# sabbirhossainujjal/LLMVoX

Hardware: AMD Instinct MI355X
Metric: speech tokens/sec (+ 24kHz audio samples/sec = 320 x tokens/s; p50 first-chunk latency) (higher is better)
Workload: dtype bf16

## Files before the change

### llmvox_amd/csrc/ar_kernels.hip

```cpp
#include "ar_plan.h"

#pragma clang fp contract(off)

namespace lvx {

#ifdef LVX_TIMING
constexpr int TS_BLOCKS = 1024;
__device__ uint64_t g_lvx_ts[16 * 4 * TS_BLOCKS * 4];
#define TS_DECL uint64_t ts_[2] = {0, 0}
#define TS_MARK(i) do { if (threadIdx.x == 0) ts_[i] = __builtin_amdgcn_s_memrealtime(); } while (0)
#define TS_SAVE(tag, layer, blk)                                                                    \
  do {                                                                                               \
    if (threadIdx.x == 0) {                                                                          \
      const uint64_t te_ = __builtin_amdgcn_s_memrealtime();                                         \
      const uint64_t hw_ = (uint64_t)__builtin_amdgcn_s_getreg((31 << 11) | 4) |                    \
                           ((uint64_t)__builtin_amdgcn_s_getreg((3 << 11) | 20) << 32);              \
      uint64_t* p_ = g_lvx_ts + ((size_t)(((tag) * 4 + (layer)) * TS_BLOCKS + min((int)(blk), TS_BLOCKS - 1))) * 4; \
      p_[0] = ts_[0]; p_[1] = ts_[1]; p_[2] = te_; p_[3] = hw_;                                      \
    }                                                                                                \
  } while (0)
#else
#define TS_DECL do {} while (0)
#define TS_MARK(i) do {} while (0)
#define TS_SAVE(tag, layer, blk) do {} while (0)
// ... 908 lines not shown
__device__ __forceinline__ void slot_update_bf16(float& m, float& l, f32x2_t (&o)[12], float sc, const uint4 (&vp)[3],
                                                 bool valid) {
  uint32_t v[12];
#pragma unroll
  for (int i = 0; i < 3; ++i) { v[4 * i] = vp[i].x; v[4 * i + 1] = vp[i].y; v[4 * i + 2] = vp[i].z; v[4 * i + 3] = vp[i].w; }
  if (!valid) return;
  const float mn = fmaxf(m, sc);
  const float alpha = __builtin_amdgcn_exp2f((m - mn) * 1.4426950408889634f);
  const float p = __builtin_amdgcn_exp2f((sc - mn) * 1.4426950408889634f);
  l = l * alpha + p;
  const f32x2_t a2 = f32x2_t{alpha, alpha}, p2 = f32x2_t{p, p};
#pragma unroll
  for (int j = 0; j < 12; ++j) {
    const f32x2_t vv = f32x2_t{__uint_as_float(v[j] << 16), __uint_as_float(v[j] & 0xffff0000u)};
    o[j] = __builtin_elementwise_fma(p2, vv, o[j] * a2);
  }
  m = mn;
}
__device__ __forceinline__ void slot_softmax_step_bf16(float& m, float& l, f32x2_t (&o)[12], const QSplit& qs,
                                                       const uint4 (&kp)[3], const uint4 (&vp)[3], bool valid) {
  slot_update_bf16(m, l, o, slot_score_bf16(qs, kp), vp, valid);
}

__device__ __forceinline__ float slot_fold_wave(float m, float& l, float (&o)[24]) {
  const float M = wave_max(m);
  const float f = (m == -INFINITY) ? 0.f : expf(m - M);
  l *= f;
#pragma unroll
  for (int i = 0; i < 24; ++i) o[i] *= f;
  return M;
}

__device__ __forceinline__ float4 q0_row_stats(const GemvArgs& a, int4 rn, int b, int lane, bool store_x);
__device__ __forceinline__ int l0_next_tok(const ArState& st, int jn, int loaded) {
  if (!st.text_plan) return 384;
  return (jn + 1 < st.plan_stride) ? min(max(loaded, 0), TEXT_VOCAB - 1) : -1;
}
__device__ __forceinline__ void lds_barrier() {
  asm volatile("s_waitcnt lgkmcnt(0)" ::: "memory");
  __builtin_amdgcn_s_barrier();
  asm volatile("" ::: "memory");
}

template <typename TKV, int DEPTH, int NW, bool QKV, bool L0>
__device__ __forceinline__ void attn_v2_body(const ArState st, int layer, int ns_max, int direct, int selcopy,
                                             const GemvArgs* a0) {
  constexpr int TK = NW * 16;
  constexpr bool SLOT = sizeof(TKV) < 4;
  static_assert(!QKV || (NW == 4 && sizeof(TKV) == 4), "the K-split c_attn: the fp32 parity mode's 4-wave blocks");
  static_assert(!L0 || (NW == 4 && SLOT && !QKV), "the fused layer-0 form: bf16 / fp8 KV in 4-wave blocks");
  constexpr bool NEWKV = QKV || L0;
  constexpr int QH = NEWKV ? (3 * HD + NW * 64 - 1) / (NW * 64) : 1;
  __shared__ float wm_s[NW], wl_s[NW];
  __shared__ float wo_s[NW][4][HD];
  __shared__ float qs_s[NEWKV ? HD : 1];
  __shared__ __attribute__((aligned(16))) TKV kvh_s[NEWKV ? 2 : 1][NEWKV ? HD : 1];
  __shared__ float sv_s[L0 ? 4 : 1], sv2_s[L0 ? 4 : 1];
  __shared__ int si_s[L0 ? 4 : 1];
  __shared__ float4 sst_s;
  const int sp = blockIdx.x, head = blockIdx.y, b = blockIdx.z;
  const int tid = threadIdx.x, wave = tid >> 6, lane = tid & 63;
  TS_DECL;
  TS_MARK(0);
  int4 rold = make_int4(-1, 0, 0, 0);
  int2 rx = make_int2(0, 0);
  bool tk = false;
  float4 lgv[L0 ? VOCAB / 1024 : 1];
  int zn[L0 ? QH : 1];
  float zg[L0 ? QH : 1], zt[L0 ? QH : 1], zp[L0 ? QH : 1];
  int jnx = 0, tnext = 384;
  int4 ri0 = make_int4(-1, 0, 0, 0);
  if constexpr (L0) {
    rold = st.rowinfo[b];
    rx = st.rowx[b];
    const unsigned pend = st.selrow[b];
    const float4* lg = reinterpret_cast<const float4*>(st.logits + (size_t)b * VOCAB);
#pragma unroll
    for (int k = 0; k < VOCAB / 1024; ++k) lgv[k] = lg[k * 256 + tid];
#pragma unroll
    for (int h = 0; h < QH; ++h) {
      const int e = min(tid + NW * 64 * h, 3 * HD - 1);
      zn[h] = (e / HD) * D + head * HD + e % HD;
      zg[h] = a0->q0_g[zn[h]];
    }
    tk = pend && rold.x >= 0;
    const int p1 = min(max(tk ? rold.y + 1 : rold.y, 0), st.max_pos - 1);
    const int t1 = tk ? rx.y : rold.z;
#pragma unroll
    for (int h = 0; h < QH; ++h) {
      zt[h] = a0->q0_text[(size_t)(t1 < 0 ? 384 : t1) * (3 * D) + zn[h]];
      zp[h] = a0->q0_pos[(size_t)p1 * (3 * D) + zn[h]];
    }
    jnx = tk ? rx.x + 1 : rx.x;
    if (st.text_plan) tnext = st.text_plan[(size_t)b * st.plan_stride + min(jnx + 1, st.plan_stride - 1)];
    ri0 = make_int4(rold.x, p1, 0, 0);
    if (rold.x < 0) {
      if (head == 0) {
        if (tid == 0) {
          st.rowinfo_n[b] = rold;
          st.rowx_n[b] = make_int2(jnx, l0_next_tok(st, jnx, tnext));
        }
        if (tid < D / 4) reinterpret_cast<float4*>(st.x + (size_t)b * D)[tid] = make_float4(0.f, 0.f, 0.f, 0.f);
      }
      return;
    }
  }
  const int4 ri = L0 ? ri0 : selcopy ? st.rowinfo_n[b] : st.rowinfo[b];
  float pq[QH][QKV ? 4 : 1];
  if constexpr (QKV) {
#pragma unroll
    for (int h = 0; h < QH; ++h) {
      const int e = min(tid + NW * 64 * h, 3 * HD - 1);
      const float* pp = st.qkvp + (size_t)b * (3 * D) + (e / HD) * D + head * HD + e % HD;
#pragma unroll
      for (int k = 0; k < 4; ++k) pq[h][k] = pp[(size_t)k * st.max_streams * (3 * D)];
    }
  }
  const bool cp = selcopy && sp == 0 && head == 0 && tid == 0;
  int jn = 0;
  if (cp) {
    jn = st.rowx_n[b].x;
    st.rowinfo[b] = ri;
    st.selrow[b] = 1u;
    if (b == 0) *st.selp = 0u;
  }
  auto copy_tail = [&]() {
    if (cp) st.rowx[b] = make_int2(jn, plan_tok(st, b, jn + 1));
  };
  const int s = ri.x;
  if (s < 0) {
    copy_tail();
    if (direct == ATTN_F32_ROWS && sp == 0 && tid < HD) st.part_o[(size_t)(b * N_HEAD + head) * NSPLIT * HD + tid] = 0.f;
    return;
  }
  const int t = ri.y + 1;
  const int ns = min(ns_max, (t + ATK - 1) / ATK);
  if (sp >= ns) return;
  const int chunk = SLOT ? (((t + ns - 1) / ns + ATK - 1) / ATK) * ATK : (t + ns - 1) / ns;
  const int k0 = sp * chunk, k1 = L0 ? t - 1 : min(t, k0 + chunk);
  const size_t base = kv_at(layer, st.kv_chunks, st.max_streams, s, head, 0);
  const size_t cstride = (size_t)st.max_streams * N_HEAD * KV_CHUNK * HD;
  const TKV* __restrict__ Kg = reinterpret_cast<const TKV*>(st.kc) + base;
  const TKV* __restrict__ Vg = reinterpret_cast<const TKV*>(st.vc) + base;
  auto krow = [&](int k) { return (size_t)(k / KV_CHUNK) * cstride + (size_t)(k % KV_CHUNK) * HD; };
  const int part = tid & 3, kq = tid >> 2;
  float q[24];
  if constexpr (!NEWKV) {
    const float* qg = st.q + (size_t)b * D + head * HD + part * 24;
#pragma unroll
    for (int i = 0; i < 24; i += 4) {
      const float4 v = *reinterpret_cast<const float4*>(qg + i);
      q[i] = v.x * 0.10206207261596575f; q[i + 1] = v.y * 0.10206207261596575f;
      q[i + 2] = v.z * 0.10206207261596575f; q[i + 3] = v.w * 0.10206207261596575f;
    }
  }
  float m = -INFINITY, l = 0.f, o[24];
#pragma unroll
  for (int i = 0; i < 24; ++i) o[i] = 0.f;
  KvPiece<TKV> kpr[DEPTH][3], vpr[DEPTH][3];
  const int klast = ((k1 - 1) / ATK) * ATK;
  auto issue = [&](int kb, KvPiece<TKV>(&kp)[3], KvPiece<TKV>(&vp)[3]) {
    if constexpr (SLOT) {
      const size_t off = (size_t)min((kb / KV_CHUNK) + (kq / KV_CHUNK), klast / KV_CHUNK) * cstride +
                         (size_t)(kq % KV_CHUNK) * HD + part * 24;
#pragma unroll
      for (int i = 0; i < 3; ++i) {
        kp[i].load(Kg + off + i * 8);
        vp[i].load(Vg + off + i * 8);
      }
      return;
    }
    const int key = min(kb + kq, k1 - 1);
// ... 51 lines not shown
    const float alpha = (m == -INFINITY) ? 0.f : expf(m - mn);
    const float p = valid ? expf(sc - mn) : 0.f;
    l = l * alpha + wave_sum(part == 0 ? p : 0.f);
#pragma unroll
    for (int i = 0; i < 24; ++i) o[i] = fmaf(valid ? p : 0.f, valid ? vf[i] : 0.f, o[i] * alpha);
    m = mn;
  };
#pragma unroll
  for (int d = 0; d < DEPTH; ++d) issue(k0 + d * TK, kpr[d], vpr[d]);
  if constexpr (QKV) {
#pragma unroll
    for (int h = 0; h < QH; ++h) {
      const int e = tid + NW * 64 * h;
      float v = 0.f;
#pragma unroll
      for (int k = 0; k < 4; ++k) v += pq[h][k];
      if (e < HD) {
        qs_s[e] = v;
      } else if (e < 3 * HD && k1 == t) {
        const int which = e / HD - 1, d = e % HD;
        TKV hv;
        if constexpr (sizeof(TKV) == 4) hv = v;
        else if constexpr (sizeof(TKV) == 2) hv = f32_to_bf16(v);
        else hv = f32_to_fp8(v);
        kvh_s[which][d] = hv;
        reinterpret_cast<TKV*>(which ? st.vc : st.kc)[base + krow(ri.y) + d] = hv;
      }
    }
    asm volatile("s_waitcnt lgkmcnt(0)" ::: "memory");
    __builtin_amdgcn_s_barrier();
    asm volatile("" ::: "memory");
#pragma unroll
    for (int i = 0; i < 24; ++i) q[i] = qs_s[part * 24 + i] * 0.10206207261596575f;
  }
  if constexpr (L0) {
    const GemvArgs& a = *a0;
    Best bt{-INFINITY, -INFINITY, 0x7fffffff};
#pragma unroll
    for (int k = 0; k < VOCAB / 1024; ++k) {
      const int i0 = (k * 256 + tid) * 4;
      bt = best_merge(bt, Best{lgv[k].x, -INFINITY, i0});
      bt = best_merge(bt, Best{lgv[k].y, -INFINITY, i0 + 1});
      bt = best_merge(bt, Best{lgv[k].z, -INFINITY, i0 + 2});
      bt = best_merge(bt, Best{lgv[k].w, -INFINITY, i0 + 3});
    }
    bt = best_wave(bt);
    if (lane == 0) { sv_s[wave] = bt.v; sv2_s[wave] = bt.v2; si_s[wave] = bt.i; }
    lds_barrier();
    int4 rn = rold;
    if (tk) {
      Best r{sv_s[0], sv2_s[0], si_s[0]};
#pragma unroll
      for (int w = 1; w < 4; ++w) r = best_merge(r, Best{sv_s[w], sv2_s[w], si_s[w]});
      r = softmax_ties(st.logits + (size_t)b * VOCAB, r, lane);
      const int sl = rold.x, p = rold.y + 1, j = rx.x;
      rn = make_int4(sl, min(p, st.max_pos - 1), rx.y, min(max(r.i, 0), VOCAB - 1));
      if (head == 0 && tid == 0) {
        if (p >= st.max_pos) atomicOr(st.err, 1);
        if (j < st.plan_stride) {
          st.tok_plan[(size_t)b * st.plan_stride + j] = r.i;
          if (st.margin_plan) st.margin_plan[(size_t)b * st.plan_stride + j] = r.v - r.v2;
        }
        st.prev[sl] = r.i;
        st.pos[sl] = p;
        st.rowstep[b] = j + 1;
      }
// ... 12 lines not shown
    lds_barrier();
    const float4 ss = sst_s;
    const float cz = rn.y == 0 ? 0.f : 1.f;
#pragma unroll
    for (int h = 0; h < QH; ++h) {
      const int e = tid + NW * 64 * h;
      const float v = ss.z * (((zt[h] + cz * zc[h]) * ss.x + zp[h]) - ss.y * zg[h]);
      if (e < HD) {
        qs_s[e] = v;
      } else if (e < 3 * HD) {
        const int which = e / HD - 1, d = e % HD;
        TKV hv;
        if constexpr (sizeof(TKV) == 2) hv = f32_to_bf16(v);
        else hv = f32_to_fp8(v);
        kvh_s[which][d] = hv;
        reinterpret_cast<TKV*>(which ? st.vc : st.kc)[base + krow(ri.y) + d] = hv;
      }
    }
    lds_barrier();
#pragma unroll
    for (int i = 0; i < 24; ++i) q[i] = qs_s[part * 24 + i] * 0.10206207261596575f;
    TS_MARK(1);
  }
  if constexpr (BF) qsplit_make(q, qsp);
  for (int kb = k0; kb < k1; kb += DEPTH * TK) {
#pragma unroll
    for (int d = 0; d < DEPTH; ++d) {
      if (DEPTH == 2 && d > 0 && kb + d * TK >= k1) break;
      tile(kb + d * TK, kpr[d], vpr[d]);
      issue(kb + (d + DEPTH) * TK, kpr[d], vpr[d]);
      if (DEPTH > 2) __builtin_amdgcn_sched_barrier(0);
    }
  }
  if constexpr (L0) {
    const bool mine = kq == (t - 1) % TK;
    KvPiece<TKV> kx[3], vx[3];
#pragma unroll
    for (int i = 0; i < 3; ++i) {
      kx[i].load(kvh_s[0] + part * 24 + i * 8);
      vx[i].load(kvh_s[1] + part * 24 + i * 8);
    }
    if constexpr (BF) {
      uint4 ku[3], vu[3];
#pragma unroll
      for (int i = 0; i < 3; ++i) { ku[i] = reinterpret_cast<const uint4&>(kx[i]); vu[i] = reinterpret_cast<const uint4&>(vx[i]); }
      slot_softmax_step_bf16(m, l, o2, qsp, ku, vu, mine);
    } else {
      float kf[24], vf[24];
#pragma unroll
      for (int i = 0; i < 3; ++i) { kx[i].get(kf + 8 * i); vx[i].get(vf + 8 * i); }
      slot_softmax_step(m, l, o, q, kf, vf, mine);
    }
    TS_SAVE(9, layer, head + N_HEAD * b);
  }
  if constexpr (BF) {
#pragma unroll
    for (int j = 0; j < 12; ++j) { o[2 * j] = o2[j].x; o[2 * j + 1] = o2[j].y; }
  }
  if constexpr (SLOT) {
    m = slot_fold_wave(m, l, o);
    l = wave_sum(part == 0 ? l : 0.f);
  }
#pragma unroll
  for (int i = 0; i < 24; ++i) {
    float v = o[i];
    v += dpp_f32<0x128>(v);
    v += dpp_f32<0x124>(v);
// ... 15 lines not shown
    float ov = 0.f, lv = 0.f;
#pragma unroll
    for (int w = 0; w < NW; ++w) {
      const float f = (wm_s[w] == -INFINITY) ? 0.f : expf(wm_s[w] - M);
      ov += f * ((wo_s[w][0][tid] + wo_s[w][1][tid]) + (wo_s[w][2][tid] + wo_s[w][3][tid]));
      lv += f * wl_s[w];
    }
    if (direct == ATTN_F32_ROWS) {
      st.part_o[(size_t)(b * N_HEAD + head) * NSPLIT * HD + tid] = ov * (1.0f / lv);
      return;
    }
    if (direct) {
      st.xn[direct == ATTN_XN_PACKED ? xfrag(b, head * HD + tid, D) : (size_t)b * D + head * HD + tid] = f32_to_bf16(ov * (1.0f / lv));
      return;
    }
    st.part_o[((size_t)(b * N_HEAD + head) * NSPLIT + sp) * HD + tid] = ov;
    if (tid == 0) {
      float* ml = st.part_ml + ((size_t)(b * N_HEAD + head) * NSPLIT + sp) * 2;
      ml[0] = M;
      ml[1] = lv;
    }
  }
}

template <typename TKV, int DEPTH, int NW, bool QKV = false>
__global__ __launch_bounds__(NW * 64) void ar_attn_v2_kernel(ArState st, int layer, int ns_max, int direct,
                                                         int selcopy) {
  attn_v2_body<TKV, DEPTH, NW, QKV, false>(st, layer, ns_max, direct, selcopy, nullptr);
}

template <typename TKV>
__global__ __launch_bounds__(256) LVX_LOADS_FIRST void ar_attn_l0_kernel(GemvArgs a, int direct) {
  attn_v2_body<TKV, 2, 4, false, true>(a.st, 0, 1, direct, 0, &a);
}

__device__ __forceinline__ void hist_store(const ArState& st, int s, int p, int tok) {
  if (st.rowstep && p < st.max_pos) st.hist[(size_t)s * st.max_pos + p] = (uint16_t)tok;
}

template <bool HIST = false>
__device__ __forceinline__ void argmax_row(const ArState& st, int b, int4 ri, float* sv, float* sv2, int* si) {
  const int tid = threadIdx.x, wave = tid >> 6, lane = tid & 63;
  const float4* lg = reinterpret_cast<const float4*>(st.logits + (size_t)b * VOCAB);
  Best bt{-INFINITY, -INFINITY, 0x7fffffff};
#pragma unroll
  for (int j = 0; j < VOCAB / 1024; ++j) {
    const float4 v = lg[j * 256 + tid];
    const int i0 = (j * 256 + tid) * 4;
    bt = best_merge(bt, Best{v.x, -INFINITY, i0});
    bt = best_merge(bt, Best{v.y, -INFINITY, i0 + 1});
    bt = best_merge(bt, Best{v.z, -INFINITY, i0 + 2});
    bt = best_merge(bt, Best{v.w, -INFINITY, i0 + 3});
  }
  bt = best_wave(bt);
  if (lane == 0) { sv[wave] = bt.v; sv2[wave] = bt.v2; si[wave] = bt.i; }
  __syncthreads();
  if (wave == 0) {
    Best r{sv[0], sv2[0], si[0]};
    for (int w = 1; w < 4; ++w) r = best_merge(r, Best{sv[w], sv2[w], si[w]});
    r = softmax_ties(st.logits + (size_t)b * VOCAB, r, lane);
    if (lane == 0) {
      argmax_commit(st, b, ri, r);
      if constexpr (HIST) hist_store(st, ri.x, ri.y, r.i);
    }
  }
}
// ... 236 lines not shown
  if (tid == 0) {
    first = min(min(wfirst[0], wfirst[1]), min(wfirst[2], wfirst[3]));
    last = max(max(wlast[0], wlast[1]), max(wlast[2], wlast[3]));
    r.i = first != 0x7fffffff ? first : max(last, 0);
    hist_store(st, s, ri.y, r.i);
    argmax_commit(st, b, ri, r);
  }
}


template <typename TW, int K, int KW, int RPW, int IN, int OUT>
static void launch_gemv(const GemvArgs& a, hipStream_t s) {
  const int rows_per_block = (4 / KW) * RPW;
  dim3 grid((a.N + rows_per_block - 1) / rows_per_block);
  constexpr int BGMAX = (K == 768) ? 16 : 4;
  if constexpr (OUT == GOUT_LOGITS_GRAN || IN == GIN_EMBED_SELECT) {
    if (a.B <= 1) hipLaunchKernelGGL((ar_gemv_kernel<TW, K, KW, RPW, 1, IN, OUT>), grid, dim3(256), 0, s, a);
    else if (a.B <= 2) hipLaunchKernelGGL((ar_gemv_kernel<TW, K, KW, RPW, 2, IN, OUT>), grid, dim3(256), 0, s, a);
    else hipLaunchKernelGGL((ar_gemv_kernel<TW, K, KW, RPW, 4, IN, OUT>), grid, dim3(256), 0, s, a);
  } else {
    if constexpr (IN == GIN_MERGE && OUT == GOUT_RESID && K == 768 && KW == 1) {
      if (a.B == 1) {
        hipLaunchKernelGGL((ar_cproj_b1_kernel<TW, RPW, NSPLIT>), grid, dim3(256), 0, s, a);
        return;
      }
    }
    if (a.B <= 1) hipLaunchKernelGGL((ar_gemv_kernel<TW, K, KW, RPW, 1, IN, OUT>), grid, dim3(256), 0, s, a);
    else if (a.B <= 2) hipLaunchKernelGGL((ar_gemv_kernel<TW, K, KW, RPW, 2, IN, OUT>), grid, dim3(256), 0, s, a);
    else if (a.B <= 4 || BGMAX == 4) hipLaunchKernelGGL((ar_gemv_kernel<TW, K, KW, RPW, 4, IN, OUT>), grid, dim3(256), 0, s, a);
    else if (a.B <= 8) hipLaunchKernelGGL((ar_gemv_kernel<TW, K, KW, RPW, (BGMAX >= 8 ? 8 : 4), IN, OUT>), grid, dim3(256), 0, s, a);
    else hipLaunchKernelGGL((ar_gemv_kernel<TW, K, KW, RPW, BGMAX, IN, OUT>), grid, dim3(256), 0, s, a);
  }
}

typedef __bf16 bf16x8_t __attribute__((ext_vector_type(8)));
typedef float f32x4_t __attribute__((ext_vector_type(4)));

__device__ __forceinline__ uint2 pack4_bf16(float4 v) {
  return make_uint2((uint32_t)f32_to_bf16(v.x) | ((uint32_t)f32_to_bf16(v.y) << 16),
                    (uint32_t)f32_to_bf16(v.z) | ((uint32_t)f32_to_bf16(v.w) << 16));
}

#ifndef LVX_YCS
#define LVX_YCS 2
#endif
constexpr int YCS = LVX_YCS;

__device__ __forceinline__ void embed_row(const GemvArgs& a, int4 ri, int lane, float4 (&v)[3], float* rden = nullptr) {
  if (ri.x < 0) {
#pragma unroll
    for (int j = 0; j < 3; ++j) v[j] = make_float4(0.f, 0.f, 0.f, 0.f);
    return;
  }
  const int p = ri.y, prev = ri.w;
  const int tok = ri.z < 0 ? 384 : ri.z;
  float4 pe[3];
  const float* wr_ = a.wpe + (size_t)p * D;
#pragma unroll
  for (int j = 0; j < 3; ++j) pe[j] = *reinterpret_cast<const float4*>(wr_ + j * 256 + lane * 4);
#pragma unroll
  for (int j = 0; j < 3; ++j) {
    const int k = j * 256 + lane * 4;
    v[j] = j == 0 ? *reinterpret_cast<const float4*>(a.text_table + (size_t)tok * TEXT_DIM + k)
                  : *reinterpret_cast<const float4*>(a.codebook + (size_t)prev * SPEECH_DIM + (k - TEXT_DIM));
  }
  if (ri.z < 0 && lane == 0) atomicOr(a.st.err, 2);
  float ss = 0.f;
#pragma unroll
  for (int j = 0; j < 3; ++j) {
// ... 397 lines not shown
  const int B = a.B;
  TS_DECL;
  TS_MARK(0);
  const bf16_t* __restrict__ X = XM == M2X_LN_AFTER ? a.st.xb : ((KTOT == 768) ? a.st.xn : a.st.hb);
  const int k0 = by * K + wave * 192 + 8 * (lane >> 4);
  constexpr int EPT = (16 * NT * 16 + NW * 64 - 1) / (NW * 64);
  static_assert((NW * 64) % (NT * 16) == 0, "one batch row per thread in the epilogue");
  int4 ripre = make_int4(-1, 0, 0, 0);
  float xpre[(OUT == M2OUT_RESID_STATS || OUT == M2OUT_RESID) ? EPT : 1];
  float gpre[(OUT == M2OUT_RESID_STATS || XM == M2X_LN_AFTER) ? EPT : 1];
  if constexpr (OUT == M2OUT_QKV) ripre = a.st.rowinfo[min(r0 + tid % (NT * 16), B - 1)];
  if constexpr (OUT == M2OUT_RESID) {
#pragma unroll
    for (int k = 0; k < EPT; ++k) {
      const int e = min(tid + k * NW * 64, 16 * NT * 16 - 1), r = e / (NT * 16), b = min(r0 + e - r * (NT * 16), B - 1);
      const int n = min(n0 + r, a.N - 1);
      float t = a.st.x[(size_t)b * D + n];
      const float* yp = a.yacc ? a.yacc + (size_t)b * YCS * D + n : a.st.x + (size_t)b * D + n;
      const int ys = a.yacc ? D : 0;
      float yc[YCS];
#pragma unroll
      for (int c = 0; c < YCS; ++c) yc[c] = yp[c * ys];
      if (a.yacc && a.add_y)
#pragma unroll
        for (int c = 0; c < YCS; ++c) t += yc[c];
      xpre[k] = t;
    }
  }
  if constexpr (OUT == M2OUT_RESID_STATS || XM == M2X_LN_AFTER) {
#pragma unroll
    for (int k = 0; k < EPT; ++k) {
      const int e = min(tid + k * NW * 64, 16 * NT * 16 - 1), r = e / (NT * 16), b = e - r * (NT * 16);
      const int n = min(n0 + r, a.N - 1);
      if constexpr (OUT == M2OUT_RESID_STATS) xpre[k] = a.st.x[(size_t)min(r0 + b, B - 1) * D + n];
      gpre[k] = OUT == M2OUT_RESID_STATS ? a.ln_w[n] : a.gsum[n];
    }
  }
  float2 sp[XM == M2X_LN_AFTER ? 12 : 1];
  if constexpr (XM == M2X_LN_AFTER) {
    const int rr = min(tid >> 2, NT * 16 - 1), q = tid & 3;
    const float2* xs = reinterpret_cast<const float2*>(a.st.xstat) + (size_t)min(r0 + rr, B - 1) * (D / 16) + q * 12;
#pragma unroll
    for (int j = 0; j < 12; ++j) sp[j] = xs[j];
    __builtin_amdgcn_sched_barrier(0);
  }
  uint4 wf[6], xf[NT][6];
  const bf16_t* wsrc = reinterpret_cast<const bf16_t*>(a.Wf) +
                       (((size_t)(n0 >> 4) * (KTOT / 32) + (by * K + wave * 192) / 32) * 64 + lane) * 8;
#pragma unroll
  for (int kk = 0; kk < 6; ++kk) wf[kk] = *reinterpret_cast<const uint4*>(wsrc + kk * 512);
#pragma unroll
  for (int t = 0; t < NT; ++t) {
    const int b = min(r0 + t * 16 + (lane & 15), B - 1);
    const bf16_t* xsrc = a.xpk ? X + ((((size_t)(r0 >> 4) + t) * (KTOT / 32) + (by * K + wave * 192) / 32) * 64 + lane) * 8
                               : X + (size_t)b * KTOT + k0;
    const int xstep = a.xpk ? 512 : 32;
#pragma unroll
    for (int kk = 0; kk < 6; ++kk) xf[t][kk] = *reinterpret_cast<const uint4*>(xsrc + kk * xstep);
  }
  __builtin_amdgcn_sched_barrier(0);
  if constexpr (XM == M2X_LN_AFTER) {
    if (tid < NT * 16 * 4) {
      const int rr = tid >> 2, q = tid & 3;
      const float2 (&p)[12] = sp;
      float mean = 0.f, m2 = 0.f;
#pragma unroll
      for (int j = 0; j < 12; ++j) {
// ... 786 lines not shown
    case OP_LM_HEAD:
      a.W = w.w_lm; a.Wf = w.f_lm; a.N = VOCAB; a.ln_w = w.lnf;
      if (p.ksplit) {
        hipLaunchKernelGGL((ar_rows_kernel<RMODE_LN_Y_F32>), dim3(B), dim3(64), 0, s, a);
        launch_f32b<768, FIN_LN_ROWS, FOUT_LOGITS>(a, s);
      } else {
        launch_f32b<768, FIN_LN, FOUT_LOGITS>(a, s);
      }
      break;
  }
}

template <typename TW>
static bool launch_op(int op, GemvArgs& a, const ArWeights& w, int l, const ArStepPlan& p, hipStream_t s) {
  if (p.path == PATH_F32B || p.path == PATH_BT) {
    if (p.path == PATH_F32B) launch_op_f32b(op, a, w, l, p, s);
    else launch_op_bt(op, a, w, l, p, s);
    return true;
  }
  const int B = p.B;
  const bool ln = p.path == PATH_MFMA_LN, mf = ln || p.path == PATH_MFMA_ROWS, fm = p.fused_mlp;
  a.xpk = p.xpk;
  a.layer = l;
  a.yacc = mf ? a.st.yacc : nullptr;
  a.yfx = fm ? a.st.yfx : nullptr;
  a.add_y = l > 0;
  switch (op) {
    case OP_QKV:
      a.W = w.w_attn[l]; a.Wf = w.f_attn[l]; a.N = 3 * D; a.ln_w = w.ln1[l];
      if (!(p.sel == SEL_ARGMAX || (mf ? p.sel == SEL_EMBED || p.sel == SEL_Q0_ROWS || (ln && p.sel == SEL_LN_GRAN)
                                       : p.sel == SEL_GRAN)))
        ar_plan_bug(p, "c_attn");
      if (l == 0 && p.l0_fused) {
      } else if (l == 0 && p.sel == SEL_LN_GRAN) {
        launch_mfma_ln<MLOUT_QKV, MLMODE_EMBED_SELECT>(a, s);
      } else if (l == 0 && p.sel == SEL_Q0_ROWS) {
        hipLaunchKernelGGL(ar_q0_rows_kernel, dim3(3 * D / 256, B), dim3(256), 0, s, a);
      } else if (l == 0 && p.sel == SEL_EMBED) {
        hipLaunchKernelGGL(ar_embed_select_kernel<>, dim3(B), dim3(256), 0, s, a);
        launch_mfma2<768, M2OUT_QKV>(a, s);
      } else if (ln) {
        if (l == 0) launch_mfma_ln<MLOUT_QKV, MLMODE_EMBED>(a, s);
        else launch_mfma_ln<MLOUT_QKV, MLMODE_LN_Y>(a, s);
      } else if (mf) {
        if (l == 0) hipLaunchKernelGGL((ar_rows_kernel<RMODE_EMBED>), dim3(B), dim3(64), 0, s, a);
        else if (l == 1 && p.l0_fused) hipLaunchKernelGGL((ar_rows_kernel<RMODE_LN_Y_COPY>), dim3(B), dim3(64), 0, s, a);
        else hipLaunchKernelGGL((ar_rows_kernel<RMODE_LN_Y>), dim3(B), dim3(64), 0, s, a);
        launch_mfma2<768, M2OUT_QKV>(a, s);
      } else if (l == 0 && p.q0_gran) {
        hipLaunchKernelGGL(ar_q0_gran_kernel, dim3(3 * D / 256), dim3(256), 0, s, a);
      } else if (l == 0 && p.sel == SEL_GRAN) {
        launch_gemv<TW, 768, 1, 2, GIN_EMBED_SELECT, GOUT_QKV>(a, s);
      } else if (l == 0) {
        launch_gemv<TW, 768, 1, 2, GIN_EMBED, GOUT_QKV>(a, s);
      } else if (fm) {
        launch_gemv<TW, 768, 1, 2, GIN_LN_Y, GOUT_QKV>(a, s);
      } else {
        launch_gemv<TW, 768, 1, 2, GIN_LN, GOUT_QKV>(a, s);
      }
      break;
    case OP_ATTN:
      if (l == 0 && p.l0_fused) {
        if (p.kv_dtype == LVX_DTYPE_BF16)
          hipLaunchKernelGGL(ar_attn_l0_kernel<bf16_t>, dim3(1, N_HEAD, B), dim3(256), 0, s, a, p.attn_direct);
        else if (p.kv_dtype == LVX_DTYPE_FP8)
          hipLaunchKernelGGL(ar_attn_l0_kernel<fp8_t>, dim3(1, N_HEAD, B), dim3(256), 0, s, a, p.attn_direct);
        else ar_plan_bug(p, "fused layer-0 attention");
        break;
      }
      launch_attn(a.st, p.kv_dtype, B, l, s, p.nsplit, p.attn_direct, p.selcopy && l == 0, false, p.attn8);
      break;
    case OP_CPROJ:
      a.W = w.w_aproj[l]; a.Wf = w.f_aproj[l]; a.N = D;
      if (mf) {
        if (!ln) a.add_y = 0;
        if (p.nsplit > 1) launch_merge_bf16(a.st, B, p.nsplit, s, a.xpk);
        a.ln_w = w.ln2[l];
        if (!ln) launch_mfma2<768, M2OUT_RESID_STATS>(a, s, true);
        else launch_mfma2<768, M2OUT_RESID>(a, s);
      } else {
        launch_gemv<TW, 768, 1, 1, GIN_MERGE, GOUT_RESID>(a, s);
      }
      break;
    case OP_FC:
      a.W = w.w_fc[l]; a.Wf = w.f_fc[l]; a.N = DFF; a.ln_w = w.ln2[l];
      if (fm) {
        const bf16_t* wfc = reinterpret_cast<const bf16_t*>(w.w_fc[l]);
        const bf16_t* wpk = reinterpret_cast<const bf16_t*>(w.w_mproj_pk[l]);
        if (B <= 1) hipLaunchKernelGGL((ar_mlp_fused_kernel<1, 16>), dim3(DFF / 16), dim3(256), 0, s, a, wfc, wpk);
        else hipLaunchKernelGGL((ar_mlp_fused_kernel<2, 16>), dim3(DFF / 16), dim3(256), 0, s, a, wfc, wpk);
      } else if (ln) {
        launch_mfma_ln<MLOUT_GELU_BF16, MLMODE_LN>(a, s);
      } else if (mf) {
        a.gsum = w.fc_gsum[l];
        launch_mfma2<768, M2OUT_GELU_BF16, M2X_LN_AFTER>(a, s);
      } else {
        launch_gemv<TW, 768, 1, 2, GIN_LN, GOUT_GELU>(a, s);
      }
      break;
    case OP_MPROJ:
      a.W = w.w_mproj[l]; a.Wf = w.f_mproj[l]; a.N = D;
      if (fm) return false;
      if (ln && YCS < YCOPIES)
        hipLaunchKernelGGL((ar_mfma2_kernel<DFF / YCS, 1, M2OUT_SPLITK, DFF>), dim3(D / 16, YCS), dim3(DFF / YCS / 192 * 64), 0, s, a);
      else if (mf) launch_mproj_split<M2OUT_SPLITK>(a, s);
      else launch_gemv<TW, 3072, 4, 2, GIN_H, GOUT_RESID>(a, s);
      break;
    case OP_LM_HEAD:
// ... 426 lines not shown
```

### llmvox_amd/csrc/ar_plan.h

```cpp
#pragma once
#include <stdio.h>
#include <stdlib.h>

#include "lvx_internal.h"

namespace lvx {

enum { OP_QKV = 0, OP_ATTN = 1, OP_CPROJ = 2, OP_FC = 3, OP_MPROJ = 4, OP_LM_HEAD = 5 };
enum { GIN_LN = 0, GIN_H = 1, GIN_MERGE = 2, GIN_EMBED = 3, GIN_LN_Y = 4, GIN_EMBED_SELECT = 5 };
enum { GOUT_QKV = 0, GOUT_RESID = 1, GOUT_GELU = 2, GOUT_LOGITS = 3, GOUT_SPLITK = 6, GOUT_LOGITS_GRAN = 9 };
enum { RMODE_LN = 0, RMODE_EMBED = 3, RMODE_LN_Y = 4, RMODE_LN_Y_F32 = 5, RMODE_EMBED_F32 = 6, RMODE_LN_Y_COPY = 7 };
enum { M2OUT_QKV = 0, M2OUT_RESID = 1, M2OUT_LOGITS = 3, M2OUT_GELU_BF16 = 5, M2OUT_SPLITK = 6, M2OUT_RESID_STATS = 7 };
enum { M2X_NONE = 0, M2X_LN_AFTER = 1 };
enum { MLOUT_QKV = 0, MLOUT_LOGITS = 3, MLOUT_GELU_BF16 = 5 };
enum { MLMODE_LN = 0, MLMODE_EMBED = 3, MLMODE_LN_Y = 4, MLMODE_EMBED_SELECT = 7 };
enum { BIN_LN = 0, BIN_ROWS = 1, BIN_EMBED = 3 };
enum { BOUT_QKV = 0, BOUT_RESID = 1, BOUT_LOGITS = 3, BOUT_GELU_BF16 = 5 };
enum { FIN_LN = 0, FIN_H = 1, FIN_MERGE = 2, FIN_EMBED = 3, FIN_ATTN_ROWS = 4, FIN_LN_ROWS = 6 };
enum { FOUT_QKV = 0, FOUT_RESID = 1, FOUT_GELU = 2, FOUT_LOGITS = 3, FOUT_SPLITK = 6 };
enum { ATTN_PARTIALS = 0, ATTN_XN = 1, ATTN_XN_PACKED = 2, ATTN_F32_ROWS = 3 };

enum ArPath { PATH_GEMV, PATH_MFMA_LN, PATH_MFMA_ROWS, PATH_BT, PATH_F32B };
enum ArSelect { SEL_ARGMAX = 0, SEL_GRAN = 1, SEL_EMBED = 2, SEL_LN_GRAN = 3, SEL_Q0_ROWS = 4, SEL_SAMPLE = 5 };
enum ArEndCommit { END_NONE, END_SELECT_FINAL, END_ARGMAX };

struct ArStepPlan {
  int B, kv_dtype;
  bool bf16, row;
  ArPath path;
  ArSelect sel;
  ArEndCommit end;
  int nsplit, attn_direct;
  bool attn8, selcopy;
  bool l0_fused;
  bool fused_mlp;
  bool q0_gran;
  int xpk;
  bool ksplit, qsplit;
};

constexpr int MFMA_BATCH_MIN = 3;
constexpr int LM8_ROWS = 8;
constexpr int ATTN_BLOCKS = 256;
inline int attn_ns_max(int B) {
  int ns = NSPLIT;
  while (ns > 1 && ns * N_HEAD * B > ATTN_BLOCKS) ns >>= 1;
  return ns;
}

[[noreturn]] inline void ar_plan_bug(const ArStepPlan& p, const char* where) {
  fprintf(stderr, "llmvox: %s: no kernel for select form %d on path %d at B = %d\n", where, (int)p.sel, (int)p.path, p.B);
  abort();
}

inline ArSelect ar_plan_select(const Opts& o, const ArStepPlan& p, bool q0) {
  if (!o.defer_select) return SEL_ARGMAX;
  if (p.path == PATH_GEMV) return p.B <= 2 ? SEL_GRAN : SEL_ARGMAX;
  if (p.B < 4) return SEL_ARGMAX;
  if (p.path == PATH_BT) return SEL_EMBED;
  if (p.path == PATH_F32B) return p.qsplit ? SEL_EMBED : SEL_ARGMAX;
  if (o.l0q && q0 && p.B <= 32) return SEL_Q0_ROWS;
  if (o.defer_select == 1 && p.path == PATH_MFMA_LN && p.B <= LM8_ROWS) return SEL_LN_GRAN;
  return SEL_EMBED;
}

inline ArStepPlan ar_plan_step(const Opts& o_, int wdtype, int kvdtype, int B, bool row, bool q0, bool sample = false) {
  sample = sample && !row;
  Opts o = o_;
  if (sample) o.defer_select = 0;
  ArStepPlan p{};
  p.B = B; p.kv_dtype = kvdtype; p.bf16 = wdtype == LVX_DTYPE_BF16; p.row = row;
  const bool batched = !row && B >= MFMA_BATCH_MIN && B <= 64;
  if (!batched || (!p.bf16 && !o.f32b)) p.path = PATH_GEMV;
  else if (!p.bf16) p.path = PATH_F32B;
  else if (o.bt && (B > 32 || o.bt == 2)) p.path = PATH_BT;
  else p.path = B <= o.ln_max ? PATH_MFMA_LN : PATH_MFMA_ROWS;
  const bool mf = p.path == PATH_MFMA_LN || p.path == PATH_MFMA_ROWS;
  p.ksplit = p.path == PATH_F32B && !(o.exp & 512);
  p.qsplit = p.ksplit && B <= 32 && !(o.exp & 1024);

  p.sel = row ? SEL_ARGMAX : sample ? SEL_SAMPLE : ar_plan_select(o, p, q0);
  p.end = p.sel == SEL_ARGMAX || p.sel == SEL_SAMPLE ? END_NONE : p.sel == SEL_GRAN ? END_SELECT_FINAL : END_ARGMAX;
  p.selcopy = p.sel == SEL_GRAN || p.sel == SEL_LN_GRAN || p.sel == SEL_Q0_ROWS;
  p.q0_gran = p.sel == SEL_GRAN && o.l0q && q0;
  p.fused_mlp = p.path == PATH_GEMV && p.bf16 && o.fuse_mlp && B <= 2;

  p.attn8 = mf && B >= 5 && (B <= 8 || (kvdtype == LVX_DTYPE_FP8 && B <= 16));
  p.nsplit = p.path == PATH_GEMV ? NSPLIT : (mf && (B > 8 || p.attn8)) ? 1 : attn_ns_max(B);
  p.l0_fused = o.l0a && p.sel == SEL_Q0_ROWS && p.nsplit == 1 && !p.attn8 && B >= 9 && kvdtype != LVX_DTYPE_F32;
  p.xpk = (p.path == PATH_MFMA_ROWS && B <= 32) ? 1 : 0;
  p.attn_direct = p.nsplit > 1 || !(mf || p.path == PATH_F32B) ? ATTN_PARTIALS
                  : p.path == PATH_F32B ? ATTN_F32_ROWS : p.xpk ? ATTN_XN_PACKED : ATTN_XN;
  return p;
}

}
```

### llmvox_amd/csrc/lvx_api.cpp

```cpp
#include <hip/hip_runtime.h>

#include <cmath>
#include <cstdio>
#include <cstdlib>
#include <algorithm>
#include <atomic>
#include <cstring>
#include <functional>
#include <map>
#include <mutex>
#include <string>
#include <tuple>
#include <vector>

#include "llmvox.h"
#include "ar_plan.h"

using namespace lvx;

namespace lvx {
static const Opts kDefaultOpts{};
static thread_local const Opts* t_opts = nullptr;
const Opts& opts() { return t_opts ? *t_opts : kDefaultOpts; }
OptScope::OptScope(const Opts* o) : prev(t_opts) { t_opts = o; }
// ... 762 lines not shown
}

int lvx_stream_position(lvx_ctx* c, int slot, int* pos_out, void* stream) {
  NEED_FINAL(c);
  if (slot < 0 || slot >= c->cfg.max_streams || !pos_out) return fail(LVX_E_ARG, "bad slot/pos_out");
  HIP_TRY(hipSetDevice(c->cfg.device));
  int32_t v[2];
  launch_err_take(c->st.err, 1, 0, c->st.err + 3, (hipStream_t)stream);
  HIP_TRY(hipMemcpyAsync(&v[0], c->st.pos + slot, 4, hipMemcpyDeviceToHost, (hipStream_t)stream));
  HIP_TRY(hipMemcpyAsync(&v[1], c->st.err + 3, 4, hipMemcpyDeviceToHost, (hipStream_t)stream));
  HIP_TRY(hipStreamSynchronize((hipStream_t)stream));
  *pos_out = v[0];
  return bits_status(v[1]);
}

int lvx_set_option(lvx_ctx* c, const char* name, int value) {
  if (!c || !name) return fail(LVX_E_ARG, "null argument");
  std::string n(name);
  std::lock_guard<std::mutex> lk(c->mu);
  Opts& o = c->opts;
  if (n == "defer_select") o.defer_select = value;
  else if (n == "fuse_mlp") o.fuse_mlp = value != 0;
  else if (n == "bt") o.bt = std::min(std::max(value, 0), 2);
  else if (n == "codec_g2") o.codec_g2 = value != 0;
  else if (n == "codec_skinny") o.codec_skinny = value != 0;
  else if (n == "codec_g3") o.codec_g3 = value != 0;
  else if (n == "codec_g3f") o.codec_g3f = value == 1 ? 1 : 2;
  else if (n == "codec_exp") o.codec_exp = value;
  else if (n == "exp") o.exp = value;
  else if (n == "f32b") o.f32b = value != 0;
  else if (n == "ln_max") o.ln_max = std::min(std::max(value, 2), 8);
  else if (n == "l0q") o.l0q = value != 0;
  else if (n == "l0a") o.l0a = value != 0;
  else return fail(LVX_E_NAME, "unknown option " + n);
  ++c->opt_epoch;
  return LVX_OK;
}

int lvx_set_capture_stream(lvx_ctx* c, void* stream) {
  if (!c) return fail(LVX_E_ARG, "null ctx");
  std::lock_guard<std::mutex> lk(c->mu);
  c->capture_stream = (hipStream_t)stream;
  return LVX_OK;
}

int lvx_set_graphs(lvx_ctx* c, int enable) {
  if (!c) return fail(LVX_E_ARG, "null ctx");
  c->use_graphs = enable != 0;
  return LVX_OK;
}

int lvx_ar_forward_row(lvx_ctx* c, int slot, int pos, const float* emb_row, float* logits, void* stream) {
  NEED_FINAL(c);
  if (slot < 0 || slot >= c->cfg.max_streams) return fail(LVX_E_ARG, "slot out of range");
  if (pos < 0 || pos >= BLOCK_SIZE)
    return fail(LVX_E_CAPACITY, "Cannot forward sequence of length " + std::to_string(pos + 1) +
                                    ", block size is only " + std::to_string(BLOCK_SIZE));
  if (pos >= c->cfg.max_positions)
    return fail(LVX_E_CAPACITY, "position " + std::to_string(pos) + " exceeds the KV capacity " +
                                    std::to_string(c->cfg.max_positions));
  if (!emb_row || !logits) return fail(LVX_E_ARG, "null emb_row/logits");
  HIP_TRY(hipSetDevice(c->cfg.device));
  const Opts o = c->opts_snapshot();
  OptScope os(&o);
  ar_launch_step(c->arw, c->st, ar_plan_step(o, c->cfg.weight_dtype, c->cfg.kv_dtype, 1, true, false), emb_row, slot,
                 pos, logits, (hipStream_t)stream);
// ... 798 lines not shown
```

### llmvox_amd/csrc/lvx_internal.h

```cpp
#pragma once
#include <hip/hip_runtime.h>
#include <stdint.h>
#include <string>

#include "lvx_common.h"
#include "llmvox.h"
#include "pcm_host.h"

namespace lvx {

constexpr int N_LAYER = 4, N_HEAD = 8, D = 768, HD = 96, DFF = 3072, VOCAB = 4096;
constexpr int TEXT_DIM = 256, SPEECH_DIM = 512, TEXT_VOCAB = 386, BLOCK_SIZE = 8192;
constexpr int NSPLIT = 16;
constexpr int KV_CHUNK = 64;
__host__ __device__ inline size_t kv_at(size_t layer, size_t chunks, size_t streams, int s, int head, int pos) {
  return (((((layer * chunks + (size_t)(pos / KV_CHUNK)) * streams + s) * 8 + head) * KV_CHUNK) + (size_t)(pos % KV_CHUNK)) * 96;
}
#ifndef LVX_YCOPIES
#define LVX_YCOPIES 4
#endif
constexpr int YCOPIES = LVX_YCOPIES;
constexpr int LM_MAX_BLOCKS = 1024;
struct Opts {
  int defer_select = 1;
  int fuse_mlp = 1;
  int bt = 1;
  int codec_g2 = 1, codec_skinny = 1, codec_g3 = 1, codec_g3f = 2;
  int codec_exp = 0;
  int exp = 0;
  int f32b = 1;
  int ln_max = 8;
  int l0q = 1;
  int l0a = 1;
};
const Opts& opts();
struct OptScope {
  explicit OptScope(const Opts* o);
  ~OptScope();
  OptScope(const OptScope&) = delete;
  OptScope& operator=(const OptScope&) = delete;
  const Opts* prev;
};

struct ArWeights {
  const float* wpe = nullptr;
  const float* text_table = nullptr;
  const float* codebook = nullptr;
  const float* ln1[N_LAYER] = {};
  const float* ln2[N_LAYER] = {};
  const float* lnf = nullptr;
  const void* w_attn[N_LAYER] = {};
  const void* w_aproj[N_LAYER] = {};
  const void* w_fc[N_LAYER] = {};
  const void* w_mproj[N_LAYER] = {};
  const void* w_mproj_pk[N_LAYER] = {};
  const float* fc_gsum[N_LAYER] = {};
  const void* w_lm = nullptr;
  const float* q0_text = nullptr;
  const float* q0_code = nullptr;
  const float* q0_pos = nullptr;
  const float* q0_g = nullptr;
  const void* f_attn[N_LAYER] = {};
  const void* f_aproj[N_LAYER] = {};
  const void* f_fc[N_LAYER] = {};
  const void* f_mproj[N_LAYER] = {};
  const void* f_lm = nullptr;
// ... 150 lines not shown
```

Before: 251,400.

## Fuse LN1 and QKV projection into attention kernel for layers 1-3

For layers above zero, when the fused layer-0 path is active, the attention kernel now computes LayerNorm of the residual row (summing the y-copies) and the c_attn projection itself. It uses MFMA bf16 tiles with a rotating weight prefetch of RT tiles, writes the new K/V into the cache, and then runs attention over history plus the new token. This removes the separate LN+QKV launch and its global round-trip of qkv. The c_proj residual epilogue now folds the y-accumulator copies into the residual so that the sum is applied there. The cost is heavier attention blocks at lower occupancy, and each head recomputes the LN redundantly.

```diff
diff --git a/llmvox_amd/csrc/ar_kernels.hip b/llmvox_amd/csrc/ar_kernels.hip
--- a/llmvox_amd/csrc/ar_kernels.hip
+++ b/llmvox_amd/csrc/ar_kernels.hip
@@ -964,6 +964,9 @@
 }
 
 __device__ __forceinline__ float4 q0_row_stats(const GemvArgs& a, int4 rn, int b, int lane, bool store_x);
+__device__ __forceinline__ uint2 pack4_bf16(float4 v);
+typedef __bf16 bf16x8_t __attribute__((ext_vector_type(8)));
+typedef float f32x4_t __attribute__((ext_vector_type(4)));
 __device__ __forceinline__ int l0_next_tok(const ArState& st, int jn, int loaded) {
   if (!st.text_plan) return 384;
   return (jn + 1 < st.plan_stride) ? min(max(loaded, 0), TEXT_VOCAB - 1) : -1;
@@ -974,14 +977,16 @@
   asm volatile("" ::: "memory");
 }
 
-template <typename TKV, int DEPTH, int NW, bool QKV, bool L0>
+template <typename TKV, int DEPTH, int NW, bool QKV, bool L0, bool LA = false, int RT = 1>
 __device__ __forceinline__ void attn_v2_body(const ArState st, int layer, int ns_max, int direct, int selcopy,
                                              const GemvArgs* a0) {
   constexpr int TK = NW * 16;
   constexpr bool SLOT = sizeof(TKV) < 4;
   static_assert(!QKV || (NW == 4 && sizeof(TKV) == 4), "the K-split c_attn: the fp32 parity mode's 4-wave blocks");
   static_assert(!L0 || (NW == 4 && SLOT && !QKV), "the fused layer-0 form: bf16 / fp8 KV in 4-wave blocks");
-  constexpr bool NEWKV = QKV || L0;
+  static_assert(!LA || (NW == 4 && SLOT && !QKV && !L0), "the fused layers form: bf16 / fp8 KV in 4-wave blocks");
+  constexpr bool NEWKV = QKV || L0 || LA;
+  constexpr bool HIST = L0 || LA;
   constexpr int QH = NEWKV ? (3 * HD + NW * 64 - 1) / (NW * 64) : 1;
   __shared__ float wm_s[NW], wl_s[NW];
   __shared__ float wo_s[NW][4][HD];
@@ -990,6 +995,8 @@
   __shared__ float sv_s[L0 ? 4 : 1], sv2_s[L0 ? 4 : 1];
   __shared__ int si_s[L0 ? 4 : 1];
   __shared__ float4 sst_s;
+  __shared__ __attribute__((aligned(16))) bf16_t xb_s[LA ? NW : 1][LA ? D : 8];
+  __shared__ float red_s[LA ? NW : 1][LA ? 3 * HD : 1];
   const int sp = blockIdx.x, head = blockIdx.y, b = blockIdx.z;
   const int tid = threadIdx.x, wave = tid >> 6, lane = tid & 63;
   TS_DECL;
@@ -1038,6 +1045,26 @@
     }
   }
   const int4 ri = L0 ? ri0 : selcopy ? st.rowinfo_n[b] : st.rowinfo[b];
+  XRow<LA ? GIN_LN_Y : GIN_LN> xr;
+  float4 gam[3];
+  uint4 wr[RT][6];
+  int2 rxn = make_int2(0, 0);
+  const uint4* wsl = nullptr;
+  const int rot = LA ? (b * 7) % 18 : 0;
+  auto la_tile = [&](int i) { const int j = i + rot; return j >= 18 ? j - 18 : j; };
+  auto la_woff = [&](int j) { return (size_t)((j / 6) * 48 + j % 6) * (D / 32) * 64; };
+  if constexpr (LA) {
+    rxn = st.rowx_n[b];
+#pragma unroll
+    for (int j = 0; j < 3; ++j) gam[j] = *reinterpret_cast<const float4*>(a0->ln_w + j * 256 + lane * 4);
+    xrow_issue(*a0, b, lane, xr);
+    wsl = reinterpret_cast<const uint4*>(a0->Wf) + ((size_t)head * 6 * (D / 32) + wave * 6) * 64 + lane;
+#pragma unroll
+    for (int i = 0; i < RT; ++i)
+#pragma unroll
+      for (int kk = 0; kk < 6; ++kk) wr[i][kk] = wsl[la_woff(la_tile(i)) + kk * 64];
+    __builtin_amdgcn_sched_barrier(0);
+  }
   float pq[QH][QKV ? 4 : 1];
   if constexpr (QKV) {
 #pragma unroll
@@ -1051,7 +1078,8 @@
   const bool cp = selcopy && sp == 0 && head == 0 && tid == 0;
   int jn = 0;
   if (cp) {
-    jn = st.rowx_n[b].x;
+    if constexpr (LA) jn = rxn.x;
+    else jn = st.rowx_n[b].x;
     st.rowinfo[b] = ri;
     st.selrow[b] = 1u;
     if (b == 0) *st.selp = 0u;
@@ -1069,7 +1097,7 @@
   const int ns = min(ns_max, (t + ATK - 1) / ATK);
   if (sp >= ns) return;
   const int chunk = SLOT ? (((t + ns - 1) / ns + ATK - 1) / ATK) * ATK : (t + ns - 1) / ns;
-  const int k0 = sp * chunk, k1 = L0 ? t - 1 : min(t, k0 + chunk);
+  const int k0 = sp * chunk, k1 = HIST ? t - 1 : min(t, k0 + chunk);
   const size_t base = kv_at(layer, st.kv_chunks, st.max_streams, s, head, 0);
   const size_t cstride = (size_t)st.max_streams * N_HEAD * KV_CHUNK * HD;
   const TKV* __restrict__ Kg = reinterpret_cast<const TKV*>(st.kc) + base;
@@ -1187,6 +1215,70 @@
     asm volatile("" ::: "memory");
 #pragma unroll
     for (int i = 0; i < 24; ++i) q[i] = qs_s[part * 24 + i] * 0.10206207261596575f;
+  }
+  if constexpr (LA) {
+    {
+      float4 v[3];
+      xrow_sum(xr, v);
+      wave_ln_regs(v, gam);
+      uint2* dst = reinterpret_cast<uint2*>(xb_s[wave]);
+#pragma unroll
+      for (int j = 0; j < 3; ++j) dst[j * 64 + lane] = pack4_bf16(v[j]);
+    }
+    asm volatile("s_waitcnt lgkmcnt(0)" ::: "memory");
+    __builtin_amdgcn_wave_barrier();
+    uint4 xf[6];
+#pragma unroll
+    for (int kk = 0; kk < 6; ++kk)
+      xf[kk] = *reinterpret_cast<const uint4*>(xb_s[wave] + (wave * 6 + kk) * 32 + 8 * (lane >> 4));
+    f32x4_t accp = f32x4_t{0.f, 0.f, 0.f, 0.f};
+#pragma unroll
+    for (int i = 0; i < 18; ++i) {
+      f32x4_t acc = f32x4_t{0.f, 0.f, 0.f, 0.f};
+#pragma unroll
+      for (int kk = 0; kk < 6; ++kk)
+        acc = __builtin_amdgcn_mfma_f32_16x16x32_bf16(__builtin_bit_cast(bf16x8_t, wr[i % RT][kk]),
+                                                      __builtin_bit_cast(bf16x8_t, xf[kk]), acc, 0, 0, 0);
+      if (i + RT < 18) {
+#pragma unroll
+        for (int kk = 0; kk < 6; ++kk)
+          wr[i % RT][kk] = wsl[la_woff(la_tile(i + RT)) + kk * 64];
+      }
+      if (i > 0 && (lane & 15) == 0) {
+#pragma unroll
+        for (int r = 0; r < 4; ++r) red_s[wave][la_tile(i - 1) * 16 + 4 * (lane >> 4) + r] = accp[r];
+      }
+      accp = acc;
+      __builtin_amdgcn_sched_barrier(0);
+    }
+    if ((lane & 15) == 0) {
+#pragma unroll
+      for (int r = 0; r < 4; ++r) red_s[wave][la_tile(17) * 16 + 4 * (lane >> 4) + r] = accp[r];
+    }
+    lds_barrier();
+#pragma unroll
+    for (int h = 0; h < QH; ++h) {
+      const int e = tid + NW * 64 * h;
+      if (e < 3 * HD) {
+        float v = 0.f;
+#pragma unroll
+        for (int w = 0; w < NW; ++w) v += red_s[w][e];
+        if (e < HD) {
+          qs_s[e] = v;
+        } else {
+          const int which = e / HD - 1, d = e % HD;
+          TKV hv;
+          if constexpr (sizeof(TKV) == 2) hv = f32_to_bf16(v);
+          else hv = f32_to_fp8(v);
+          kvh_s[which][d] = hv;
+          reinterpret_cast<TKV*>(which ? st.vc : st.kc)[base + krow(ri.y) + d] = hv;
+        }
+      }
+    }
+    lds_barrier();
+#pragma unroll
+    for (int i = 0; i < 24; ++i) q[i] = qs_s[part * 24 + i] * 0.10206207261596575f;
+    TS_MARK(1);
   }
   if constexpr (L0) {
     const GemvArgs& a = *a0;
@@ -1265,7 +1357,7 @@
       if (DEPTH > 2) __builtin_amdgcn_sched_barrier(0);
     }
   }
-  if constexpr (L0) {
+  if constexpr (HIST) {
     const bool mine = kq == (t - 1) % TK;
     KvPiece<TKV> kx[3], vx[3];
 #pragma unroll
@@ -1347,6 +1439,15 @@
 template <typename TKV>
 __global__ __launch_bounds__(256) LVX_LOADS_FIRST void ar_attn_l0_kernel(GemvArgs a, int direct) {
   attn_v2_body<TKV, 2, 4, false, true>(a.st, 0, 1, direct, 0, &a);
+}
+
+#ifndef LVX_LA_RT
+#define LVX_LA_RT 3
+#endif
+template <typename TKV>
+__global__ __launch_bounds__(256) __attribute__((amdgpu_waves_per_eu(1, 2))) void ar_attn_la_kernel(GemvArgs a, int direct,
+                                                                                                    int selcopy) {
+  attn_v2_body<TKV, 2, 4, false, false, true, LVX_LA_RT>(a.st, a.layer, 1, direct, selcopy, &a);
 }
 
 __device__ __forceinline__ void hist_store(const ArState& st, int s, int p, int tok) {
@@ -1649,9 +1750,6 @@
     else hipLaunchKernelGGL((ar_gemv_kernel<TW, K, KW, RPW, BGMAX, IN, OUT>), grid, dim3(256), 0, s, a);
   }
 }
-
-typedef __bf16 bf16x8_t __attribute__((ext_vector_type(8)));
-typedef float f32x4_t __attribute__((ext_vector_type(4)));
 
 __device__ __forceinline__ uint2 pack4_bf16(float4 v) {
   return make_uint2((uint32_t)f32_to_bf16(v.x) | ((uint32_t)f32_to_bf16(v.y) << 16),
@@ -2115,7 +2213,19 @@
     for (int k = 0; k < EPT; ++k) {
       const int e = min(tid + k * NW * 64, 16 * NT * 16 - 1), r = e / (NT * 16), b = e - r * (NT * 16);
       const int n = min(n0 + r, a.N - 1);
-      if constexpr (OUT == M2OUT_RESID_STATS) xpre[k] = a.st.x[(size_t)min(r0 + b, B - 1) * D + n];
+      if constexpr (OUT == M2OUT_RESID_STATS) {
+        const int br = min(r0 + b, B - 1);
+        float t = a.st.x[(size_t)br * D + n];
+        const float* yp = a.yacc ? a.yacc + (size_t)br * YCOPIES * D + n : a.st.x + (size_t)br * D + n;
+        const int ys = a.yacc ? D : 0;
+        float yc[YCOPIES];
+#pragma unroll
+        for (int c = 0; c < YCOPIES; ++c) yc[c] = yp[c * ys];
+        if (a.yacc && a.add_y)
+#pragma unroll
+          for (int c = 0; c < YCOPIES; ++c) t += yc[c];
+        xpre[k] = t;
+      }
       gpre[k] = OUT == M2OUT_RESID_STATS ? a.ln_w[n] : a.gsum[n];
     }
   }
@@ -2968,6 +3078,7 @@
                                        : p.sel == SEL_GRAN)))
         ar_plan_bug(p, "c_attn");
       if (l == 0 && p.l0_fused) {
+      } else if (l > 0 && p.la_fused) {
       } else if (l == 0 && p.sel == SEL_LN_GRAN) {
         launch_mfma_ln<MLOUT_QKV, MLMODE_EMBED_SELECT>(a, s);
       } else if (l == 0 && p.sel == SEL_Q0_ROWS) {
@@ -3004,12 +3115,21 @@
         else ar_plan_bug(p, "fused layer-0 attention");
         break;
       }
+      if (l > 0 && p.la_fused) {
+        a.Wf = w.f_attn[l]; a.ln_w = w.ln1[l];
+        if (p.kv_dtype == LVX_DTYPE_BF16)
+          hipLaunchKernelGGL(ar_attn_la_kernel<bf16_t>, dim3(1, N_HEAD, B), dim3(256), 0, s, a, p.attn_direct, (int)(l == 1));
+        else if (p.kv_dtype == LVX_DTYPE_FP8)
+          hipLaunchKernelGGL(ar_attn_la_kernel<fp8_t>, dim3(1, N_HEAD, B), dim3(256), 0, s, a, p.attn_direct, (int)(l == 1));
+        else ar_plan_bug(p, "fused layers attention");
+        break;
+      }
       launch_attn(a.st, p.kv_dtype, B, l, s, p.nsplit, p.attn_direct, p.selcopy && l == 0, false, p.attn8);
       break;
     case OP_CPROJ:
       a.W = w.w_aproj[l]; a.Wf = w.f_aproj[l]; a.N = D;
       if (mf) {
-        if (!ln) a.add_y = 0;
+        if (!ln) a.add_y = p.la_fused && l > 0;
         if (p.nsplit > 1) launch_merge_bf16(a.st, B, p.nsplit, s, a.xpk);
         a.ln_w = w.ln2[l];
         if (!ln) launch_mfma2<768, M2OUT_RESID_STATS>(a, s, true);
diff --git a/llmvox_amd/csrc/ar_plan.h b/llmvox_amd/csrc/ar_plan.h
--- a/llmvox_amd/csrc/ar_plan.h
+++ b/llmvox_amd/csrc/ar_plan.h
@@ -37,6 +37,7 @@
   bool q0_gran;
   int xpk;
   bool ksplit, qsplit;
+  bool la_fused;
 };
 
 constexpr int MFMA_BATCH_MIN = 3;
@@ -88,6 +89,7 @@
   p.attn8 = mf && B >= 5 && (B <= 8 || (kvdtype == LVX_DTYPE_FP8 && B <= 16));
   p.nsplit = p.path == PATH_GEMV ? NSPLIT : (mf && (B > 8 || p.attn8)) ? 1 : attn_ns_max(B);
   p.l0_fused = o.l0a && p.sel == SEL_Q0_ROWS && p.nsplit == 1 && !p.attn8 && B >= 9 && kvdtype != LVX_DTYPE_F32;
+  p.la_fused = o.laf && p.l0_fused;
   p.xpk = (p.path == PATH_MFMA_ROWS && B <= 32) ? 1 : 0;
   p.attn_direct = p.nsplit > 1 || !(mf || p.path == PATH_F32B) ? ATTN_PARTIALS
                   : p.path == PATH_F32B ? ATTN_F32_ROWS : p.xpk ? ATTN_XN_PACKED : ATTN_XN;
diff --git a/llmvox_amd/csrc/lvx_api.cpp b/llmvox_amd/csrc/lvx_api.cpp
--- a/llmvox_amd/csrc/lvx_api.cpp
+++ b/llmvox_amd/csrc/lvx_api.cpp
@@ -818,6 +818,7 @@
   else if (n == "ln_max") o.ln_max = std::min(std::max(value, 2), 8);
   else if (n == "l0q") o.l0q = value != 0;
   else if (n == "l0a") o.l0a = value != 0;
+  else if (n == "laf") o.laf = value != 0;
   else return fail(LVX_E_NAME, "unknown option " + n);
   ++c->opt_epoch;
   return LVX_OK;
diff --git a/llmvox_amd/csrc/lvx_internal.h b/llmvox_amd/csrc/lvx_internal.h
--- a/llmvox_amd/csrc/lvx_internal.h
+++ b/llmvox_amd/csrc/lvx_internal.h
@@ -32,6 +32,7 @@
   int ln_max = 8;
   int l0q = 1;
   int l0a = 1;
+  int laf = 1;
 };
 const Opts& opts();
 struct OptScope {
```

Result: faster. 256,800, median of 6 (+2.1%).
